# xyzy/jubatus

Hardware: AMD Instinct MI355X
Metric: train_samples_per_sec (higher is better)
Workload: dtype fp32

## Files before the change

jubatus_amd/csrc/hip/jb_device.hpp:

```cpp
#pragma once
#include <hip/hip_runtime.h>
#include <stdint.h>

namespace jb {

constexpr uint64_t kFnvOffset = 0xcbf29ce484222325ull;
constexpr uint64_t kFnvPrime = 0x100000001b3ull;

__device__ __forceinline__ uint64_t fnv_bytes(uint64_t h, const uint8_t* p, int n) {
  for (int i = 0; i < n; ++i) {
    h ^= (uint64_t)p[i];
    h *= kFnvPrime;
  }
  return h;
}

__device__ __forceinline__ uint64_t fnv_byte(uint64_t h, uint8_t b) {
  h ^= (uint64_t)b;
  return h * kFnvPrime;
}

__device__ __forceinline__ int64_t hash_to_index(uint64_t h, uint64_t H) {
  h ^= h >> 29;
  h *= 0xbf58476d1ce4e5b9ull;
  h ^= h >> 32;
  return (int64_t)__umul64hi(h, H);
}

struct Reader {
  const uint8_t* p;
  const uint8_t* end;
  bool ok;
  __device__ __forceinline__ bool need(int64_t n) {
    if (!ok || end - p < n) { ok = false; return false; }
    return true;
  }
  __device__ __forceinline__ uint32_t be16() { uint32_t v = ((uint32_t)p[0] << 8) | p[1]; p += 2; return v; }
  __device__ __forceinline__ uint32_t be32() {
    uint32_t v = ((uint32_t)p[0] << 24) | ((uint32_t)p[1] << 16) | ((uint32_t)p[2] << 8) | p[3];
    p += 4; return v;
  }
  __device__ __forceinline__ uint64_t be64() { uint64_t hi = be32(); uint64_t lo = be32(); return (hi << 32) | lo; }

  __device__ int64_t array_len() {
    if (!need(1)) return -1;
    uint8_t t = *p++;
    if ((t & 0xf0) == 0x90) return t & 0x0f;
    if (t == 0xdc) { if (!need(2)) return -1; return be16(); }
    if (t == 0xdd) { if (!need(4)) return -1; return be32(); }
    ok = false; return -1;
  }
  __device__ bool raw(const uint8_t** s, int* n) {
    if (!need(1)) return false;
    uint8_t t = *p++;
    int64_t len;
    if ((t & 0xe0) == 0xa0) len = t & 0x1f;
    else if (t == 0xd9 || t == 0xc4) { if (!need(1)) return false; len = *p++; }
    else if (t == 0xda || t == 0xc5) { if (!need(2)) return false; len = be16(); }
    else if (t == 0xdb || t == 0xc6) { if (!need(4)) return false; len = be32(); }
    else { ok = false; return false; }
    if (!need(len)) return false;
    *s = p; *n = (int)len; p += len;
    return true;
  }
  __device__ bool number(double* out) {
    if (!need(1)) return false;
    uint8_t t = *p++;
    if (t <= 0x7f) { *out = (double)t; return true; }
    if (t >= 0xe0) { *out = (double)(int8_t)t; return true; }
    switch (t) {
      case 0xcc: if (!need(1)) return false; *out = (double)(*p++); return true;
      case 0xcd: if (!need(2)) return false; *out = (double)be16(); return true;
      case 0xce: if (!need(4)) return false; *out = (double)be32(); return true;
      case 0xcf: if (!need(8)) return false; *out = (double)be64(); return true;
      case 0xd0: if (!need(1)) return false; *out = (double)(int8_t)(*p++); return true;
      case 0xd1: if (!need(2)) return false; *out = (double)(int16_t)be16(); return true;
      case 0xd2: if (!need(4)) return false; *out = (double)(int32_t)be32(); return true;
      case 0xd3: if (!need(8)) return false; *out = (double)(int64_t)be64(); return true;
      case 0xca: { if (!need(4)) return false; uint32_t u = be32(); *out = (double)__uint_as_float(u); return true; }
      case 0xcb: {
        if (!need(8)) return false;
        uint64_t u = be64();
        *out = __longlong_as_double((long long)u);
        return true;
      }
      default: ok = false; return false;
    }
  }
};

template <class T>
__device__ __forceinline__ void sys_store(T* p, T v) {
  __hip_atomic_store(p, v, __ATOMIC_RELAXED, __HIP_MEMORY_SCOPE_SYSTEM);
}
__device__ __forceinline__ void sys_stores_block_done() {
  asm volatile("s_waitcnt vmcnt(0)" ::: "memory");
  __syncthreads();
}

__device__ __forceinline__ float wave_sum(float v) {
#pragma unroll
  for (int off = 32; off > 0; off >>= 1) v += __shfl_xor(v, off, 64);
  return v;
}

enum : int {
  kDppXor1 = 0xB1,
  kDppXor2 = 0x4E,
  kDppRowRor8 = 0x128,
  kDppHalfMirror = 0x141,
  kDppMirror = 0x140,
};

template <int CTRL>
__device__ __forceinline__ float dpp_f(float v) {
  return __int_as_float(__builtin_amdgcn_update_dpp(0, __float_as_int(v), CTRL, 0xF, 0xF, false));
}
template <int CTRL>
__device__ __forceinline__ int dpp_i(int v) {
  return __builtin_amdgcn_update_dpp(0, v, CTRL, 0xF, 0xF, false);
}

__device__ __forceinline__ float partner16_f(float v, int lane) {
  auto r = __builtin_amdgcn_permlane16_swap(__float_as_uint(v), __float_as_uint(v), false, false);
  return __uint_as_float(((lane >> 4) & 1) ? r[0] : r[1]);
}
__device__ __forceinline__ int partner16_i(int v, int lane) {
  auto r = __builtin_amdgcn_permlane16_swap((unsigned)v, (unsigned)v, false, false);
  return (int)(((lane >> 4) & 1) ? r[0] : r[1]);
}
__device__ __forceinline__ float partner32_f(float v, int lane) {
  auto r = __builtin_amdgcn_permlane32_swap(__float_as_uint(v), __float_as_uint(v), false, false);
  return __uint_as_float(lane >= 32 ? r[0] : r[1]);
}
__device__ __forceinline__ int partner32_i(int v, int lane) {
  auto r = __builtin_amdgcn_permlane32_swap((unsigned)v, (unsigned)v, false, false);
  return (int)(lane >= 32 ? r[0] : r[1]);
}

__device__ __forceinline__ float row16_sum(float v) {
  v += dpp_f<kDppXor1>(v);
  v += dpp_f<kDppXor2>(v);
  v += dpp_f<kDppHalfMirror>(v);
  v += dpp_f<kDppMirror>(v);
  return v;
}

__device__ __forceinline__ float wave_sum_fast(float v, int lane) {
  v = row16_sum(v);
  v += partner16_f(v, lane);
  v += partner32_f(v, lane);
  return v;
}

}
```

jubatus_amd/csrc/hip/jb_linear.hpp:

```cpp
#pragma once
#include "jb_device.hpp"

namespace jb {

__device__ __forceinline__ float ld_agent(const float* p) {
  return __hip_atomic_load(p, __ATOMIC_RELAXED, __HIP_MEMORY_SCOPE_AGENT);
}

using bf16_t = uint16_t;

__device__ __forceinline__ uint32_t jb_mix32(uint32_t a, uint32_t b) {
  uint32_t h = a * 0x9E3779B1u ^ (b + 0x7F4A7C15u) * 0x85EBCA77u;
  h ^= h >> 15;
  h *= 0x2C1B3C6Du;
  h ^= h >> 12;
  h *= 0x297A2D39u;
  h ^= h >> 15;
  return h;
}

__device__ __forceinline__ float bf16_f(uint32_t b) { return __uint_as_float(b << 16); }

__device__ __forceinline__ uint32_t f_bf16_sr(float v, uint32_t r) {
  const uint32_t u = __float_as_uint(v);
  if ((u & 0x7f800000u) == 0x7f800000u) return (u >> 16) | ((u & 0xffffu) ? 0x40u : 0u);
  const uint32_t t = u + (r & 0xffffu);
  return t >> 16;
}

__device__ __forceinline__ float ldw(const float* p) { return ld_agent(p); }
__device__ __forceinline__ float ldw(const bf16_t* p) {
  const uint32_t* w = reinterpret_cast<const uint32_t*>((uintptr_t)p & ~(uintptr_t)3);
  const uint32_t v = __hip_atomic_load(w, __ATOMIC_RELAXED, __HIP_MEMORY_SCOPE_AGENT);
  return ((uintptr_t)p & 2) ? __uint_as_float(v & 0xffff0000u) : __uint_as_float(v << 16);
}
__device__ __forceinline__ void stw(float* p, float v, uint32_t) { *p = v; }
__device__ __forceinline__ void stw(bf16_t* p, float v, uint32_t r) { *p = (bf16_t)f_bf16_sr(v, r); }
__device__ __forceinline__ void addw(float* p, float d, uint32_t) { atomicAdd(p, d); }
__device__ __forceinline__ void addw(bf16_t* p, float d, uint32_t r) {
  uint32_t* w = reinterpret_cast<uint32_t*>((uintptr_t)p & ~(uintptr_t)3);
  const int sh = ((uintptr_t)p & 2) ? 16 : 0;
  uint32_t old = __hip_atomic_load(w, __ATOMIC_RELAXED, __HIP_MEMORY_SCOPE_AGENT);
  for (;;) {
    const float cur = bf16_f((old >> sh) & 0xffffu);
    const uint32_t nb = f_bf16_sr(cur + d, r);
    const uint32_t nw = (old & ~(0xffffu << sh)) | (nb << sh);
    if (nw == old) return;
    const uint32_t seen = atomicCAS(w, old, nw);
    if (seen == old) return;
    old = seen;
    r = jb_mix32(r, seen);
  }
}

enum Method : int { PERCEPTRON = 0, PA = 1, PA1 = 2, PA2 = 3, CW = 4, AROW = 5, NHERD = 6 };
enum UpdateMode : int { kExact = 0, kAtomic = 1, kHogwild = 2, kSerial = 3 };

__device__ __forceinline__ bool step_coeffs(int method, float margin, float var, float nrm,
                                            bool has_l, float C, float* tau, float* beta) {
  switch (method) {
    case PERCEPTRON:
      if (margin <= 0.f) { *tau = 1.f; *beta = 0.f; return true; }
      return false;
    case PA: case PA1: case PA2: {
      const float loss = 1.f - margin;
      if (!(loss > 0.f && nrm > 0.f)) return false;
      const float sq = (has_l ? 2.f : 1.f) * nrm;
      if (method == PA) *tau = loss / sq;
      else if (method == PA1) *tau = fminf(C, loss / sq);
      else *tau = loss / (sq + 0.5f / C);
      *beta = 0.f;
      return true;
    }
    case CW: {
      if (!(var > 0.f)) return false;
      const float phi = C;
      const float b = 1.f + 2.f * phi * margin;
      const float disc = b * b - 8.f * phi * (margin - phi * var);
      const float gamma = (-b + sqrtf(fmaxf(disc, 0.f))) / (4.f * phi * var);
      if (!(gamma > 0.f)) return false;
      *tau = gamma; *beta = 2.f * gamma * phi;
      return true;
    }
    case AROW:
      if (!(margin < 1.f)) return false;
      *beta = 1.f / (var + 1.f / C);
      *tau = (1.f - margin) * *beta;
      return true;
    case NHERD: {
      if (!(margin < 1.f)) return false;
      *tau = (1.f - margin) / (var + 1.f / C);
      const float cv = 1.f + C * var;
      *beta = (C * C * var + 2.f * C) / (cv * cv);
      return true;
    }
    default: return false;
  }
}

__device__ __forceinline__ float dprec(int method, float beta, float x, float s) {
  const float bx2 = beta * x * x;
  return method == CW ? bx2 : bx2 / (1.f - bx2 * s);
}

template <int LC>
struct Lanes {
  static constexpr int LW = LC >= 64 ? 64 : LC;
  static constexpr int G = 64 / LW;
  static constexpr int K = LC >= 64 ? LC / 64 : 1;
};

template <int LC, typename WT>
__device__ __forceinline__ void sample_scores(const int32_t* __restrict__ fidx,
                                              const float* __restrict__ fval, int64_t beg,
                                              int n, const WT* W, int lane, float (&acc)[Lanes<LC>::K]) {
  using L = Lanes<LC>;
  const int g = lane / L::LW;
  const int l0 = lane % L::LW;
#pragma unroll
  for (int k = 0; k < L::K; ++k) acc[k] = 0.f;
  for (int j = g; j < n; j += L::G) {
    const int32_t idx = fidx[beg + j];
    const float x = fval[beg + j];
    if (idx >= 0) {
      const WT* wr = W + (int64_t)idx * LC + l0;
#pragma unroll
      for (int k = 0; k < L::K; ++k) acc[k] += x * ldw(wr + 64 * k);
    }
  }
#pragma unroll
  for (int off = L::LW; off < 64; off <<= 1) {
#pragma unroll
    for (int k = 0; k < L::K; ++k) acc[k] += __shfl_xor(acc[k], off, 64);
  }
}

template <int LW>
__device__ __forceinline__ void argmax_wrong(float& best, int& bl) {
#pragma unroll
  for (int off = 1; off < LW; off <<= 1) {
    const float ob = __shfl_xor(best, off, 64);
    const int ol = __shfl_xor(bl, off, 64);
    if (ol >= 0 && (bl < 0 || ob > best || (ob == best && ol < bl))) { best = ob; bl = ol; }
  }
}

template <int LC, int MODE, typename WT>
__device__ __forceinline__ void apply_feature(WT* W, float* P, int32_t idx, float x, int y,
                                              int lstar, bool use_s, int method, float tau,
                                              float beta, float a, float b, float wy, float wl,
                                              uint32_t rnd) {
  const int64_t row = (int64_t)idx * LC;
  const float dwy = use_s ? tau * a * x : tau * x;
  const float dwl = use_s ? -tau * b * x : -tau * x;
  if (MODE == kAtomic) {
    addw(W + row + y, dwy, jb_mix32((uint32_t)(row + y), rnd));
    if (lstar >= 0) addw(W + row + lstar, dwl, jb_mix32((uint32_t)(row + lstar), rnd));
    if (use_s) {
      atomicAdd(P + row + y, dprec(method, beta, x, a));
      if (lstar >= 0) atomicAdd(P + row + lstar, dprec(method, beta, x, b));
    }
  } else {
    stw(W + row + y, wy + dwy, jb_mix32((uint32_t)(row + y), rnd));
    if (lstar >= 0) stw(W + row + lstar, wl + dwl, jb_mix32((uint32_t)(row + lstar), rnd));
    if (use_s) {
      P[row + y] = 1.f / a + dprec(method, beta, x, a);
      if (lstar >= 0) P[row + lstar] = 1.f / b + dprec(method, beta, x, b);
    }
  }
}

template <int LC, int MODE, typename WT>
__device__ __forceinline__ bool general_sample(const int32_t* __restrict__ fidx,
                                               const float* __restrict__ fval, int64_t beg, int n,
                                               int y, WT* W, float* P, const bool (&act)[Lanes<LC>::K],
                                               int lane, int method, float C,
                                               uint8_t* __restrict__ touched) {
  using L = Lanes<LC>;
  const int l0 = lane % L::LW;
  const bool use_s = method >= CW;
  float acc[L::K];
  sample_scores<LC>(fidx, fval, beg, n, W, lane, acc);
  float sy = 0.f, best = -INFINITY;
  int bl = -1;
#pragma unroll
  for (int k = 0; k < L::K; ++k) {
    const int l = l0 + 64 * k;
// ... 59 lines not shown
```

jubatus_amd/csrc/hip/linear.hip:

```cpp
#include "jb_linear.hpp"

namespace jb {

template <int LC, int MODE, typename WT>
__global__ __launch_bounds__(256) void linear_train_wide_kernel(
    const int64_t* __restrict__ row_ptr, const int32_t* __restrict__ fidx,
    const float* __restrict__ fval, const int32_t* __restrict__ labels,
    const int64_t* __restrict__ stream_ptr, int nstreams, WT* W, float* P,
    const int32_t* __restrict__ active, int method, float C,
    unsigned long long* __restrict__ stats, uint8_t* __restrict__ touched) {
  using L = Lanes<LC>;
  const int lane = threadIdx.x & 63;
  const int wid = (blockIdx.x * blockDim.x + threadIdx.x) >> 6;
  if (wid >= nstreams) return;
  bool act[L::K];
#pragma unroll
  for (int k = 0; k < L::K; ++k) act[k] = active[lane % L::LW + 64 * k] != 0;
  unsigned n_upd = 0, n_valid = 0;
  for (int64_t s = stream_ptr[wid]; s < stream_ptr[wid + 1]; ++s) {
    const int y = labels[s];
    if (y < 0 || y >= LC) continue;
    ++n_valid;
    const int64_t beg = row_ptr[s];
    if (general_sample<LC, MODE, WT>(fidx, fval, beg, (int)(row_ptr[s + 1] - beg), y, W, P, act, lane,
                                 method, C, touched))
      ++n_upd;
    if (MODE == kExact) asm volatile("s_waitcnt vmcnt(0)" ::: "memory");
  }
  if (stats != nullptr && lane == 0 && n_valid > 0) {
    atomicAdd(stats, (unsigned long long)n_upd);
    atomicAdd(stats + 1, (unsigned long long)n_valid);
  }
}

#ifndef JB_KREP
#define JB_KREP 8
#endif
constexpr int kRep = JB_KREP;

template <int LC>
struct Hot {
  static constexpr int E = 512;
  static constexpr int R = (E / LC) < 64 ? (E / LC) : 64;
  static constexpr int T = 128;
};

__device__ __forceinline__ int hot_find(const int32_t* hK, const int32_t* hS, int32_t idx) {
  if (idx < 0) return -1;
  uint32_t h = ((uint32_t)idx * 0x9E3779B1u) >> 25;
  for (int p = 0; p < 128; ++p) {
    const int32_t k = hK[h];
    if (k == idx) return hS[h];
    if (k < 0) return -1;
    h = (h + 1) & 127;
  }
  return -1;
}

template <int LC, int NW>
struct HotMerge {
  static constexpr int KQ = 2 * Hot<LC>::E / 64 / NW;
  float d[KQ];
  float own[KQ];
  float oth[KQ][kRep - 1];
  bool pending = false;

  template <int E>
  __device__ __forceinline__ void issue(const float* rep, int rr, bool use_s, int nent,
                                        float (*hA)[E], int wv, int lane) {
#pragma unroll
    for (int k = 0; k < KQ; ++k) {
      const int q = wv + NW * k;
      const int t = q & 1;
      const int e = (q >> 1) * 64 + lane;
      if (e < nent && (t == 0 || use_s)) {
        float* sh = const_cast<float*>(rep) + (int64_t)(rr * 2 + t) * E + e;
        d[k] = atomicExch(&hA[t][e], 0.f);
        own[k] = d[k] != 0.f ? atomicAdd(sh, d[k]) : ld_agent(sh);
#pragma unroll
        for (int j = 0; j < kRep - 1; ++j) {
          const int r = j < rr ? j : j + 1;
          oth[k][j] = ld_agent(rep + (int64_t)(r * 2 + t) * E + e);
        }
      }
    }
    pending = true;
  }

  template <int E>
  __device__ __forceinline__ void finish(bool use_s, int nent, float (*hV)[E], float (*hB)[E],
                                         float* hD, int wv, int lane) {
    if (!pending) return;
#pragma unroll
    for (int k = 0; k < KQ; ++k) {
      const int q = wv + NW * k;
      const int t = q & 1;
      const int e = (q >> 1) * 64 + lane;
      if (e < nent && (t == 0 || use_s)) {
        float S = own[k] + d[k];
#pragma unroll
        for (int j = 0; j < kRep - 1; ++j) S += oth[k][j];
        const float others = S - hB[t][e] - d[k];
        atomicAdd(&hV[t][e], others);
        if (t == 1) hD[e] = others;
        hB[t][e] = S;
      }
    }
    pending = false;
  }
};

template <int LC>
__global__ __launch_bounds__(256) void hot_fold_kernel(float* W, float* P, int use_s,
                                                       const int32_t* __restrict__ hot_rows,
                                                       const int32_t* __restrict__ hot_n,
                                                       float* __restrict__ rep,
                                                       uint8_t* __restrict__ touched) {
  constexpr int E = Hot<LC>::E;
  const int nh = min(*hot_n, Hot<LC>::R);
  const int i = blockIdx.x * blockDim.x + threadIdx.x;
  const int e = i % E;
  const int t = i / E;
  if (e >= nh * LC || t > 1 || (t == 1 && !use_s)) return;
  float s = 0.f;
#pragma unroll
  for (int r = 0; r < kRep; ++r) {
    float* p = rep + (int64_t)(r * 2 + t) * E + e;
    s += *p;
    *p = 0.f;
  }
  const int32_t row = hot_rows[e / LC];
  float* T = t == 0 ? W : P;
  if (s != 0.f) T[(int64_t)row * LC + (e % LC)] += s;
  if (touched != nullptr && t == 0 && e % LC == 0) touched[row] = 1;
}

template <int LC>
struct Pipe {
  static_assert(LC <= 64, "pipelined path covers label capacities up to 64");
  static constexpr int G = 64 / LC;
  static constexpr int F = LC <= 32 ? 32 : 16;
  static constexpr int U = F / G;
};

__device__ __forceinline__ int64_t readlane64(int64_t v, int i) {
  const int lo = __builtin_amdgcn_readlane((int)(uint32_t)(uint64_t)v, i);
  const int hi = __builtin_amdgcn_readlane((int)((uint64_t)v >> 32), i);
  return (int64_t)(((uint64_t)(uint32_t)hi << 32) | (uint32_t)lo);
}

__device__ __forceinline__ float readlane_f(float v, int i) {
  return __int_as_float(__builtin_amdgcn_readlane(__float_as_int(v), i));
}
// ... 288 lines not shown
      const float nrm = wave_sum_fast(x2s, lane);
      float tau = 0.f, beta = 0.f;
      upd = step_coeffs(method, margin, var, nrm, lstar >= 0, C, &tau, &beta);
      if (upd) ++n_upd;
      if (upd && mine) {
        dwy = use_s ? tau * a * x_s : tau * x_s;
        dwl = use_s ? -tau * b * x_s : -tau * x_s;
        if (use_s) {
          dpy = dprec(method, beta, x_s, a);
          dpl = lstar >= 0 ? dprec(method, beta, x_s, b) : 0.f;
        }
      }
      if (MODE == kAtomic && use_s && upd) {
        bool dup = false;
        for (int j = 0; j < n_s; ++j) {
          const int32_t ij = __builtin_amdgcn_readlane(idx_s, j);
          dup |= mine && j != lane && ij == idx_s;
        }
        tau_s = tau;
        ser = mine && !dup;
        if (ser && !(HOT && hs_s >= 0)) {
          const int64_t row = (int64_t)idx_s * LC;
          dwy = tau * x_s / atomicAdd(P + row + y_s, dpy);
          if (lstar >= 0) dwl = -tau * x_s / atomicAdd(P + row + lstar, dpl);
          p_done = true;
        }
      }
    }
    if (early) {
      gather_commit<LC>(sW[wv][c1], sP[wv][c1], use_s, n1, g, l0, vmask, gw, gp);
      if (upd) {
        float fwy = 0.f, fwl = 0.f, fpy = 0.f, fpl = 0.f;
        const bool kv = lane < n1 && idx1 >= 0 && hs1 < 0;
        for (int j = 0; j < n_s; ++j) {
          const int32_t ij = __builtin_amdgcn_readlane(idx_s, j);
          const bool hit = kv && ij == idx1;
          if (__builtin_amdgcn_ballot_w64(hit)) {
            const float ay = readlane_f(dwy, j);
            const float al = readlane_f(dwl, j);
            const float by = readlane_f(dpy, j);
            const float bq = readlane_f(dpl, j);
            if (hit) { fwy += ay; fwl += al; fpy += by; fpl += bq; }
          }
        }
        __builtin_amdgcn_wave_barrier();
        if (kv && (fwy != 0.f || fwl != 0.f || fpy != 0.f || fpl != 0.f)) {
          float* nw = sW[wv][c1] + lane * LC;
          float* np = sP[wv][c1] + lane * LC;
          nw[y_s] += fwy;
          if (lstar >= 0) nw[lstar] += fwl;
          if (use_s) {
            np[y_s] += fpy;
            if (lstar >= 0) np[lstar] += fpl;
          }
        }
      }
      __builtin_amdgcn_wave_barrier();
    }
    JB_CONSUME(idx2);
    JB_CONSUME(x2);
    const int hs2 = (HOT && nent > 0) ? hot_find(hK, hS, idx2) : -1;
    bool skip = false;
    if (MODE != kAtomic && upd) {
      float cy = 0.f, cl = 0.f, qy = 0.f, ql = 0.f;
      const bool plain = mine && hs_s < 0;
      for (int j = 0; j < n_s; ++j) {
        const int32_t ij = __builtin_amdgcn_readlane(idx_s, j);
        const bool same = plain && ij == idx_s && j != lane;
        if (__builtin_amdgcn_ballot_w64(same)) {
          const float ay = readlane_f(dwy, j);
          const float al = readlane_f(dwl, j);
          const float by = readlane_f(dpy, j);
          const float bq = readlane_f(dpl, j);
          if (same) {
            if (j < lane) skip = true;
            else { cy += ay; cl += al; qy += by; ql += bq; }
          }
        }
      }
      dwy += cy; dwl += cl; dpy += qy; dpl += ql;
    }
    if (upd && mine && !skip) {
      if (HOT && hs_s >= 0) {
        const int hb = hs_s * LC;
        if (use_s) {
          const float p0 = atomicAdd(&hV[1][hb + y_s], dpy);
          atomicAdd(&hA[1][hb + y_s], dpy);
          if (MODE == kAtomic && ser) dwy = tau_s * x_s / (p0 + hD[hb + y_s]);
          if (lstar >= 0) {
            const float q0 = atomicAdd(&hV[1][hb + lstar], dpl);
            atomicAdd(&hA[1][hb + lstar], dpl);
            if (MODE == kAtomic && ser) dwl = -tau_s * x_s / (q0 + hD[hb + lstar]);
          }
        }
        atomicAdd(&hV[0][hb + y_s], dwy);
        atomicAdd(&hA[0][hb + y_s], dwy);
        if (lstar >= 0) {
          atomicAdd(&hV[0][hb + lstar], dwl);
          atomicAdd(&hA[0][hb + lstar], dwl);
        }
      } else {
        const int64_t row = (int64_t)idx_s * LC;
        const uint32_t ry = jb_mix32((uint32_t)(row + y_s), (uint32_t)s);
        const uint32_t rl = jb_mix32((uint32_t)(row + lstar), (uint32_t)s);
        if (MODE == kAtomic) {
          addw(W + row + y_s, dwy, ry);
          if (lstar >= 0) addw(W + row + lstar, dwl, rl);
          if (use_s && !p_done) {
            atomicAdd(P + row + y_s, dpy);
            if (lstar >= 0) atomicAdd(P + row + lstar, dpl);
          }
        } else {
          stw(W + row + y_s, wy + dwy, ry);
          if (lstar >= 0) stw(W + row + lstar, wl + dwl, rl);
          if (use_s) {
            P[row + y_s] = py + dpy;
            if (lstar >= 0) P[row + lstar] = pl + dpl;
          }
        }
        if (touched != nullptr) touched[idx_s] = 1;
      }
    }
    if (MODE == kExact && (upd || general_s)) asm volatile("s_waitcnt vmcnt(0)" ::: "memory");
    if (pipe1 && !early) {
      if (MODE != kExact) asm volatile("s_waitcnt vmcnt(0)" ::: "memory");
      vmask = gather_issue<LC, WT>(W, P, use_s, sI[wv][c1], n1, g, l0, gw, gp);
      gather_commit<LC>(sW[wv][c1], sP[wv][c1], use_s, n1, g, l0, vmask, gw, gp);
    }
    put_features<LC>(sI[wv][c], sX[wv][c], idx2, hs2, x2, n2, lane);
    __builtin_amdgcn_wave_barrier();
    staged = pipe1;
    idx_s = idx1; x_s = x1; n_s = n1; y_s = y1; hs_s = hs1;
    idx1 = idx2; x1 = x2; n1 = n2; y1 = y2; hs1 = hs2;
  }
  if constexpr (HOT) mrg.template finish<HE>(use_s, nent, hV, hB, hD, wv, lane);
  }
  if (stats != nullptr && lane == 0 && n_valid > 0) {
    atomicAdd(stats, (unsigned long long)n_upd);
    atomicAdd(stats + 1, (unsigned long long)n_valid);
  }
  if (HOT) {
    __syncthreads();
    for (int e = threadIdx.x; e < nent; e += blockDim.x) {
      const float dw = hA[0][e];
      if (dw != 0.f) atomicAdd(hot_rep + (int64_t)(rr * 2) * HE + e, dw);
      if (use_s) {
        const float dp = hA[1][e];
        if (dp != 0.f) atomicAdd(hot_rep + (int64_t)(rr * 2 + 1) * HE + e, dp);
      }
    }
  }
}

template <int LC, typename WT>
__global__ __launch_bounds__(256) void linear_classify_kernel(
    const int64_t* __restrict__ row_ptr, const int32_t* __restrict__ fidx,
    const float* __restrict__ fval, int n_samples, const WT* W, float* __restrict__ out) {
  using L = Lanes<LC>;
  const int lane = threadIdx.x & 63;
  const int s = (blockIdx.x * blockDim.x + threadIdx.x) >> 6;
  if (s >= n_samples) return;
  const int64_t beg = row_ptr[s];
  const int n = (int)(row_ptr[s + 1] - beg);
  float acc[L::K];
  sample_scores<LC>(fidx, fval, beg, n, W, lane, acc);
  if (lane < L::LW) {
#pragma unroll
    for (int k = 0; k < L::K; ++k) out[(int64_t)s * LC + lane + 64 * k] = acc[k];
  }
}

__global__ void scale_kernel(float* __restrict__ p, int64_t n, float a) {
  const int64_t tid = (int64_t)blockIdx.x * blockDim.x + threadIdx.x;
  const int64_t stride = (int64_t)gridDim.x * blockDim.x * 4;
  const int64_t n4 = n & ~(int64_t)3;
  for (int64_t i = tid * 4; i < n4; i += stride) {
    float4 v = *reinterpret_cast<float4*>(p + i);
    v.x *= a; v.y *= a; v.z *= a; v.w *= a;
    *reinterpret_cast<float4*>(p + i) = v;
  }
  if (tid < n - n4) p[n4 + tid] *= a;
}

__global__ void mix_apply_kernel(float* __restrict__ w, const float* __restrict__ red,
                                 const float* __restrict__ loc, int64_t n, float inv_n) {
  const int64_t tid = (int64_t)blockIdx.x * blockDim.x + threadIdx.x;
  const int64_t stride = (int64_t)gridDim.x * blockDim.x;
  const int64_t n4 = n >> 2;
  float4* w4 = reinterpret_cast<float4*>(w);
  const float4* r4 = reinterpret_cast<const float4*>(red);
  const float4* l4 = reinterpret_cast<const float4*>(loc);
  for (int64_t i = tid; i < n4; i += stride) {
    float4 a = w4[i];
    const float4 r = r4[i], l = l4[i];
    a.x += r.x * inv_n - l.x; a.y += r.y * inv_n - l.y;
    a.z += r.z * inv_n - l.z; a.w += r.w * inv_n - l.w;
    w4[i] = a;
  }
  for (int64_t i = (n4 << 2) + tid; i < n; i += stride) w[i] += red[i] * inv_n - loc[i];
}

}

extern "C" int64_t jb_serial_scratch_bytes(int64_t n_max);
extern "C" int jb_serial_prepare(const int64_t* row_ptr, const int32_t* fidx, const float* fval,
                                 const int32_t* labels, const int64_t* stream_ptr, int nstreams,
                                 int64_t n_max, float* W, float* S, const int32_t* active, int LC,
                                 int method, float C, unsigned long long* stats, uint8_t* touched,
                                 void* scratch, int64_t scratch_bytes, int bail_after,
                                 hipStream_t stream);
extern "C" int jb_stepper_train(const int64_t* row_ptr, const int32_t* fidx, const float* fval,
                                const int32_t* labels, const int64_t* range, float* W, float* P,
                                const int32_t* active, int LC, int method, float C, unsigned long long* stats,
                                uint8_t* touched, int* err, hipStream_t stream);
extern "C" int jb_stepper_enabled();
constexpr int kSerialBail = 128;

namespace jb {

__global__ void stream_span_kernel(const int64_t* __restrict__ sp, int nstreams,
                                   int64_t* __restrict__ out) {
  if (threadIdx.x == 0) {
    out[0] = sp[0];
    out[1] = sp[nstreams];
  }
}

template <typename WT, int L, int M>
void launch_train(const int64_t* row_ptr, const int32_t* fidx, const float* fval,
                  const int32_t* labels, const int64_t* stream_ptr, int nstreams, WT* W, float* S,
                  const int32_t* active, int method, float C, bool hot, int hot_nw,
                  const int32_t* hot_rows, const int32_t* hot_n, float* hot_rep, int merge_every,
                  unsigned long long* stats, uint8_t* touched, hipStream_t stream) {
  const int threads = 256;
  const int blocks = (nstreams * 64 + threads - 1) / threads;
  const int hblocks = (nstreams + hot_nw - 1) / hot_nw;
#define JB_PIPE(H, NWV, B)                                                                      \
  hipLaunchKernelGGL((linear_train_pipe_kernel<L, M, H, NWV, WT>), dim3(B), dim3(64 * NWV), 0,  \
                     stream, row_ptr, fidx, fval, labels, stream_ptr, nstreams, W, S, active,   \
                     method, C, hot_rows, hot_n, hot_rep, merge_every, stats, touched);
  if constexpr (L <= 64) {
    if constexpr (M != kExact && sizeof(WT) == 4) {
      if (hot) {
        if constexpr (L <= 16) {
          if (hot_nw == 16) { JB_PIPE(true, 16, hblocks) return; }
        }
        if (hot_nw == 4) { JB_PIPE(true, 4, hblocks) }
        else { JB_PIPE(true, 8, hblocks) }
        return;
      }
    }
    JB_PIPE(false, 4, blocks)
  } else {
    hipLaunchKernelGGL((linear_train_wide_kernel<L, M, WT>), dim3(blocks), dim3(threads), 0, stream,
                       row_ptr, fidx, fval, labels, stream_ptr, nstreams, W, S, active, method, C,
                       stats, touched);
  }
#undef JB_PIPE
}

template <typename WT, int L>
void launch_train_mode(int mode, const int64_t* row_ptr, const int32_t* fidx, const float* fval,
                       const int32_t* labels, const int64_t* stream_ptr, int nstreams, WT* W,
                       float* S, const int32_t* active, int method, float C, bool hot, int hot_nw,
                       const int32_t* hot_rows, const int32_t* hot_n, float* hot_rep,
                       int merge_every, unsigned long long* stats, uint8_t* touched,
                       hipStream_t stream) {
#define JB_ARGS row_ptr, fidx, fval, labels, stream_ptr, nstreams, W, S, active, method, C, hot, \
                hot_nw, hot_rows, hot_n, hot_rep, merge_every, stats, touched, stream
  if (mode == kAtomic) launch_train<WT, L, kAtomic>(JB_ARGS);
  else if (mode == kHogwild) launch_train<WT, L, kHogwild>(JB_ARGS);
  else launch_train<WT, L, kExact>(JB_ARGS);
#undef JB_ARGS
}

}

template <typename WT>
static int linear_train_impl(const int64_t* row_ptr, const int32_t* fidx, const float* fval,
                             const int32_t* labels, const int64_t* stream_ptr, int nstreams,
                             WT* W, float* S, const int32_t* active, int LC, int method, float C,
                             int mode, const int32_t* hot_rows, const int32_t* hot_n,
                             float* hot_rep, int merge_every, int hot_waves,
                             unsigned long long* stats, uint8_t* touched, int64_t n_max,
                             void* scratch, int64_t scratch_bytes, hipStream_t stream) {
  if (nstreams <= 0) return 0;
  if (mode == jb::kSerial && nstreams == 1) mode = jb::kExact;
  if (mode == jb::kExact && nstreams > 1) mode = jb::kSerial;
  if (mode == jb::kSerial) {
    if constexpr (sizeof(WT) == 4) {
      const int rc = jb_serial_prepare(row_ptr, fidx, fval, labels, stream_ptr, nstreams, n_max,
                                       W, S, active, LC, method, C, stats, touched, scratch,
                                       scratch_bytes, kSerialBail, stream);
      if (rc != 0) return rc;
    } else {
      if (scratch == nullptr || scratch_bytes < 16) return -3;
      hipLaunchKernelGGL(jb::stream_span_kernel, dim3(1), dim3(64), 0, stream, stream_ptr,
                         nstreams, (int64_t*)scratch);
    }
    stream_ptr = (const int64_t*)scratch;
    nstreams = 1;
    mode = jb::kExact;
    hot_rows = nullptr;
  }
  if constexpr (sizeof(WT) == 4) {
    if (mode == jb::kExact && nstreams == 1 && LC <= 64 && jb_stepper_enabled())
      return jb_stepper_train(row_ptr, fidx, fval, labels, stream_ptr, W, S, active, LC, method, C,
                              stats, touched, nullptr, stream);
  }
  const bool hot = sizeof(WT) == 4 && hot_rows != nullptr && hot_n != nullptr &&
                   hot_rep != nullptr && mode != jb::kExact && LC <= 64;
  if (merge_every < 1) merge_every = 1;
  const int hot_nw = (hot_waves == 16 && LC <= 16) ? 16 : (hot_waves == 4 ? 4 : 8);
#define JB_TRAIN(L)                                                                             \
  jb::launch_train_mode<WT, L>(mode, row_ptr, fidx, fval, labels, stream_ptr, nstreams, W, S,   \
                               active, method, C, hot, hot_nw, hot_rows, hot_n, hot_rep,        \
                               merge_every, stats, touched, stream);
  JB_LC_DISPATCH(LC, JB_TRAIN)
#undef JB_TRAIN
  if constexpr (sizeof(WT) == 4) {
    if (hot) {
#define JB_FOLD(L)                                                                            \
  hipLaunchKernelGGL((jb::hot_fold_kernel<(L <= 64 ? L : 64)>), dim3(2 * jb::Hot<64>::E / 256), \
                     dim3(256), 0, stream, W, S, method >= jb::CW ? 1 : 0, hot_rows, hot_n,     \
                     hot_rep, touched);
      JB_LC_DISPATCH(LC, JB_FOLD)
#undef JB_FOLD
    }
  }
  return (int)hipGetLastError();
}

extern "C" int jb_linear_train(const int64_t* row_ptr, const int32_t* fidx, const float* fval,
                               const int32_t* labels, const int64_t* stream_ptr, int nstreams,
                               float* W, float* S, const int32_t* active, int LC, int method,
                               float C, int mode, const int32_t* hot_rows, const int32_t* hot_n,
                               float* hot_rep, int merge_every, int hot_waves,
                               unsigned long long* stats, uint8_t* touched, int64_t n_max,
                               void* scratch, int64_t scratch_bytes, hipStream_t stream) {
  return linear_train_impl<float>(row_ptr, fidx, fval, labels, stream_ptr, nstreams, W, S, active,
                                  LC, method, C, mode, hot_rows, hot_n, hot_rep, merge_every,
                                  hot_waves, stats, touched, n_max, scratch, scratch_bytes, stream);
}

extern "C" int jb_linear_train_bf16(const int64_t* row_ptr, const int32_t* fidx,
                                    const float* fval, const int32_t* labels,
                                    const int64_t* stream_ptr, int nstreams, jb::bf16_t* W,
                                    float* S, const int32_t* active, int LC, int method, float C,
                                    int mode, unsigned long long* stats, uint8_t* touched,
                                    void* scratch, int64_t scratch_bytes, hipStream_t stream) {
  return linear_train_impl<jb::bf16_t>(row_ptr, fidx, fval, labels, stream_ptr, nstreams, W, S,
                                       active, LC, method, C, mode, nullptr, nullptr, nullptr, 1,
                                       8, stats, touched, 0, scratch, scratch_bytes, stream);
}

extern "C" int64_t jb_hot_rep_bytes() { return (int64_t)jb::kRep * 2 * jb::Hot<8>::E * 4; }

template <typename WT>
static int linear_classify_impl(const int64_t* row_ptr, const int32_t* fidx, const float* fval,
                                int n_samples, const WT* W, int LC, float* out,
                                hipStream_t stream) {
  if (n_samples <= 0) return 0;
  const int threads = 256;
  const int blocks = (n_samples * 64 + threads - 1) / threads;
#define JB_CLS(L)                                                                           \
  hipLaunchKernelGGL((jb::linear_classify_kernel<L, WT>), dim3(blocks), dim3(threads), 0, \
                     stream, row_ptr, fidx, fval, n_samples, W, out);
  JB_LC_DISPATCH(LC, JB_CLS)
#undef JB_CLS
  return (int)hipGetLastError();
}

extern "C" int jb_linear_classify(const int64_t* row_ptr, const int32_t* fidx, const float* fval,
                                  int n_samples, const float* W, int LC, float* out,
                                  hipStream_t stream) {
  return linear_classify_impl<float>(row_ptr, fidx, fval, n_samples, W, LC, out, stream);
}

extern "C" int jb_linear_classify_bf16(const int64_t* row_ptr, const int32_t* fidx,
                                       const float* fval, int n_samples, const jb::bf16_t* W,
                                       int LC, float* out, hipStream_t stream) {
  return linear_classify_impl<jb::bf16_t>(row_ptr, fidx, fval, n_samples, W, LC, out, stream);
}

extern "C" int jb_scale(float* p, int64_t n, float a, hipStream_t stream) {
  if (n <= 0) return 0;
  const int threads = 256;
  int64_t blocks = (n / 4 + threads - 1) / threads;
  if (blocks > 4096) blocks = 4096;
  if (blocks < 1) blocks = 1;
  hipLaunchKernelGGL(jb::scale_kernel, dim3((unsigned)blocks), dim3(threads), 0, stream, p, n, a);
  return (int)hipGetLastError();
}

extern "C" int jb_mix_apply(float* w, const float* red, const float* loc, int64_t n, float inv_n,
                            hipStream_t stream) {
  if (n <= 0) return 0;
  if (((uintptr_t)w | (uintptr_t)red | (uintptr_t)loc) & 15) return -2;
  const int threads = 256;
  int64_t blocks = (n / 4 + threads - 1) / threads;
  if (blocks > 8192) blocks = 8192;
  if (blocks < 1) blocks = 1;
  hipLaunchKernelGGL(jb::mix_apply_kernel, dim3((unsigned)blocks), dim3(threads), 0, stream, w, red,
                     loc, n, inv_n);
  return (int)hipGetLastError();
}
```

Baseline: 269.5 million.

## Add software-pipelined block-per-stream training kernel for wide label capacities

Adds a new training kernel for label capacities above 64 that assigns one block per stream. Each thread owns one or more label columns, and weight rows for the next sample are gathered into registers while the current sample is scored and updated. Updates to rows shared between consecutive samples are forwarded through shared memory rather than re-read, and per-sample metadata is staged in windows. It becomes the default path, with the old wide kernel kept behind an environment variable; the cost is heavy register use from the F×K arrays and one block per stream, which may limit occupancy.

```diff
diff --git a/jubatus_amd/csrc/hip/jb_device.hpp b/jubatus_amd/csrc/hip/jb_device.hpp
--- a/jubatus_amd/csrc/hip/jb_device.hpp
+++ b/jubatus_amd/csrc/hip/jb_device.hpp
@@ -153,4 +153,14 @@
   return v;
 }
 
+__device__ __forceinline__ float wave_sum_xor(float v, int lane) {
+  v += partner32_f(v, lane);
+  v += partner16_f(v, lane);
+  v += dpp_f<kDppRowRor8>(v);
+  v += dpp_f<0x124>(v);
+  v += dpp_f<kDppXor2>(v);
+  v += dpp_f<kDppXor1>(v);
+  return v;
 }
+
+}
diff --git a/jubatus_amd/csrc/hip/jb_linear.hpp b/jubatus_amd/csrc/hip/jb_linear.hpp
--- a/jubatus_amd/csrc/hip/jb_linear.hpp
+++ b/jubatus_amd/csrc/hip/jb_linear.hpp
@@ -33,6 +33,14 @@
   const uint32_t* w = reinterpret_cast<const uint32_t*>((uintptr_t)p & ~(uintptr_t)3);
   const uint32_t v = __hip_atomic_load(w, __ATOMIC_RELAXED, __HIP_MEMORY_SCOPE_AGENT);
   return ((uintptr_t)p & 2) ? __uint_as_float(v & 0xffff0000u) : __uint_as_float(v << 16);
+}
+__device__ __forceinline__ float ldw_at(const float* W, int64_t base, int col) {
+  return ld_agent(W + base + col);
+}
+__device__ __forceinline__ float ldw_at(const bf16_t* W, int64_t base, int col) {
+  const uint32_t* w = reinterpret_cast<const uint32_t*>(W) + (base >> 1) + (col >> 1);
+  const uint32_t v = __hip_atomic_load(w, __ATOMIC_RELAXED, __HIP_MEMORY_SCOPE_AGENT);
+  return (col & 1) ? __uint_as_float(v & 0xffff0000u) : __uint_as_float(v << 16);
 }
 __device__ __forceinline__ void stw(float* p, float v, uint32_t) { *p = v; }
 __device__ __forceinline__ void stw(bf16_t* p, float v, uint32_t r) { *p = (bf16_t)f_bf16_sr(v, r); }
diff --git a/jubatus_amd/csrc/hip/linear.hip b/jubatus_amd/csrc/hip/linear.hip
--- a/jubatus_amd/csrc/hip/linear.hip
+++ b/jubatus_amd/csrc/hip/linear.hip
@@ -1,4 +1,7 @@
 #include "jb_linear.hpp"
+
+#include <cstdlib>
+#include <cstring>
 
 namespace jb {
 
@@ -593,6 +596,383 @@
   }
 }
 
+template <int LC>
+struct WidePipe {
+  static_assert(LC > 64, "label capacities up to 64 run linear_train_pipe_kernel");
+  static constexpr int T = LC <= 512 ? LC : 256;
+  static constexpr int K = LC / T;
+  static constexpr int NW = T / 64;
+  static constexpr int F = 16;
+  static constexpr int WIN = 64;
+};
+
+template <int LC, int MODE, typename WT>
+__global__ __launch_bounds__(WidePipe<LC>::T) void linear_train_wide_pipe_kernel(
+    const int64_t* __restrict__ row_ptr, const int32_t* __restrict__ fidx,
+    const float* __restrict__ fval, const int32_t* __restrict__ labels,
+    const int64_t* __restrict__ stream_ptr, int nstreams, WT* W, float* P,
+    const int32_t* __restrict__ active, int method, float C,
+    unsigned long long* __restrict__ stats, uint8_t* __restrict__ touched) {
+  using Q = WidePipe<LC>;
+  constexpr int T = Q::T, K = Q::K, NW = Q::NW, F = Q::F, WIN = Q::WIN;
+  static_assert(F == 16, "the match maps below split a wave into 4 x 16 lanes");
+  __shared__ int64_t dRP[WIN + 1];
+  __shared__ int32_t dLab[WIN];
+  __shared__ int32_t sI[2][F];
+  __shared__ float sX[2][F];
+  __shared__ int32_t sN[2];
+  __shared__ int32_t sY[2];
+  __shared__ int64_t sBeg[2];
+  __shared__ float sBest[NW];
+  __shared__ int32_t sBl[NW];
+  __shared__ float sSy;
+  __shared__ float sRow[4][F];
+  __shared__ float sInc[4][F];
+  __shared__ float sFwd[4][F];
+  __shared__ uint32_t sM[2];
+  __shared__ int32_t sUpd;
+  const int tid = threadIdx.x;
+  const int lane = tid & 63;
+  const int wv = tid >> 6;
+  const bool use_s = method >= CW;
+  if ((int)blockIdx.x >= nstreams) return;
+  const int64_t s_beg = stream_ptr[blockIdx.x];
+  const int64_t s_end = stream_ptr[blockIdx.x + 1];
+  if (s_beg >= s_end) return;
+  bool act[K];
+#pragma unroll
+  for (int k = 0; k < K; ++k) act[k] = active[tid + T * k] != 0;
+
+  int64_t wb = s_beg;
+  auto load_window = [&]() {
+    for (int i = tid; i <= WIN; i += T) {
+      dRP[i] = (wb + i <= s_end) ? row_ptr[wb + i] : 0;
+      if (i < WIN) dLab[i] = (wb + i < s_end) ? labels[wb + i] : -1;
+    }
+    __syncthreads();
+  };
+  auto fetch = [&](int64_t t, int& n, int& y, int64_t& beg, int32_t& idx, float& x) {
+    n = 0; y = -1; beg = 0; idx = -1; x = 0.f;
+    if (t < s_end) {
+      const int i = (int)(t - wb);
+      beg = dRP[i];
+      n = (int)(dRP[i + 1] - beg);
+      y = dLab[i];
+      if (lane < n && lane < F) {
+        idx = fidx[beg + lane];
+        x = fval[beg + lane];
+      }
+    }
+  };
+  auto put = [&](int slot, int n, int y, int64_t beg, int32_t idx, float x) {
+    const bool v = lane < F && lane < n && idx >= 0;
+    const uint32_t m = (uint32_t)__builtin_amdgcn_ballot_w64(v);
+    if (lane < F) {
+      sI[slot][lane] = v ? idx : -1;
+      sX[slot][lane] = v ? x : 0.f;
+    }
+    if (lane == 0) { sN[slot] = n; sY[slot] = y; sBeg[slot] = beg; sM[slot] = m; }
+  };
+  float cw[F][K], cp[F][K];
+  float gw[F][K], gp[F][K];
+  auto gather_rows = [&](const int32_t* si) {
+    int64_t rows[F];
+#pragma unroll
+    for (int j = 0; j < F; ++j) {
+      const int32_t idx = __builtin_amdgcn_readfirstlane(si[j]);
+      rows[j] = (int64_t)(idx >= 0 ? idx : 0) * LC;
+    }
+    if (use_s) {
+#pragma unroll
+      for (int j = 0; j < F; ++j) {
+#pragma unroll
+        for (int k = 0; k < K; ++k) {
+          gw[j][k] = ldw_at(W, rows[j], tid + T * k);
+          gp[j][k] = ld_agent(P + rows[j] + (tid + T * k));
+        }
+      }
+    } else {
+#pragma unroll
+      for (int j = 0; j < F; ++j) {
+#pragma unroll
+        for (int k = 0; k < K; ++k) {
+          gw[j][k] = ldw_at(W, rows[j], tid + T * k);
+          gp[j][k] = 1.f;
+        }
+      }
+    }
+  };
+  auto take_rows = [&](int slot) {
+    const uint32_t m = __builtin_amdgcn_readfirstlane(sM[slot]);
+#pragma unroll
+    for (int j = 0; j < F; ++j) {
+      const bool v = (m >> j) & 1u;
+#pragma unroll
+      for (int k = 0; k < K; ++k) {
+        cw[j][k] = v ? gw[j][k] : 0.f;
+        cp[j][k] = v ? gp[j][k] : 1.f;
+      }
+    }
+  };
+
+  load_window();
+  if (wv == 0) {
+    int n, y; int64_t beg; int32_t idx; float x;
+    fetch(s_beg, n, y, beg, idx, x);
+    put(0, n, y, beg, idx, x);
+    fetch(s_beg + 1, n, y, beg, idx, x);
+    put(1, n, y, beg, idx, x);
+  }
+  __syncthreads();
+  bool staged = sN[0] <= F;
+#pragma unroll
+  for (int j = 0; j < F; ++j) {
+#pragma unroll
+    for (int k = 0; k < K; ++k) { cw[j][k] = 0.f; cp[j][k] = 1.f; gw[j][k] = 0.f; gp[j][k] = 1.f; }
+  }
+  if (staged) {
+    gather_rows(sI[0]);
+    take_rows(0);
+  }
+  unsigned n_upd = 0, n_valid = 0;
+
+  for (int64_t s = s_beg; s < s_end; ++s) {
+    const int c = (int)((s - s_beg) & 1);
+    const int c1 = c ^ 1;
+    if (s + 3 - wb > WIN) {
+      wb = s;
+      load_window();
+    }
+    const int n_s = sN[c];
+    const int y_s = sY[c];
+    const int n1 = sN[c1];
+    const bool valid_s = y_s >= 0 && y_s < LC;
+    const bool general_s = valid_s && !staged;
+    const bool pipe1 = s + 1 < s_end && n1 <= F;
+    const bool early = pipe1 && !general_s;
+    int n2 = 0, y2 = -1;
+    int64_t beg2 = 0;
+    int32_t idx2 = -1;
+    float x2 = 0.f;
+    if (wv == 0) fetch(s + 2, n2, y2, beg2, idx2, x2);
+    if (early) gather_rows(sI[c1]);
+    bool upd = false;
+    int lstar = -1;
+    if (general_s) {
+      __syncthreads();
+      if (wv == 0) {
+        using L = Lanes<LC>;
+        bool actg[L::K];
+#pragma unroll
+        for (int k = 0; k < L::K; ++k) actg[k] = active[lane + 64 * k] != 0;
+        if (general_sample<LC, MODE, WT>(fidx, fval, sBeg[c], n_s, y_s, W, P, actg, lane, method, C,
+                                         touched))
+          ++n_upd;
+        ++n_valid;
+        asm volatile("s_waitcnt vmcnt(0)" ::: "memory");
+      }
+#pragma unroll
+      for (int j = 0; j < F; ++j) {
+#pragma unroll
+        for (int k = 0; k < K; ++k) { cw[j][k] = 0.f; cp[j][k] = 1.f; gw[j][k] = 0.f; gp[j][k] = 1.f; }
+      }
+    } else if (valid_s) {
+      float acc[K];
+#pragma unroll
+      for (int k = 0; k < K; ++k) acc[k] = 0.f;
+#pragma unroll
+      for (int j = 0; j < F; ++j) {
+        const float x = readlane_f(sX[c][j], 0);
+#pragma unroll
+        for (int k = 0; k < K; ++k) acc[k] += x * cw[j][k];
+      }
+      float best = -INFINITY;
+      int bl = -1;
+#pragma unroll
+      for (int k = 0; k < K; ++k) {
+        const int l = tid + T * k;
+        if (l == y_s) sSy = acc[k];
+        if (act[k] && l != y_s && acc[k] > best) { best = acc[k]; bl = l; }
+      }
+      group_argmax<64>(best, bl, lane);
+      if (lane == 0) { sBest[wv] = best; sBl[wv] = bl; }
+      __syncthreads();
+      best = sBest[0];
+      bl = sBl[0];
+#pragma unroll
+      for (int w = 1; w < NW; ++w) {
+        const float ob = sBest[w];
+        const int ol = sBl[w];
+        if (ol >= 0 && (bl < 0 || ob > best || (ob == best && ol < bl))) { best = ob; bl = ol; }
+      }
+      lstar = bl;
+      const float margin = sSy - (lstar >= 0 ? best : 0.f);
+#pragma unroll
+      for (int k = 0; k < K; ++k) {
+        const int l = tid + T * k;
+        if (l == y_s || l == lstar) {
+          const int t = l == y_s ? 0 : 1;
+#pragma unroll
+          for (int j = 0; j < F; ++j) {
+            sRow[t][j] = cw[j][k];
+            sRow[2 + t][j] = cp[j][k];
+          }
+        }
+      }
+      __syncthreads();
+      if (wv == 0) {
+        ++n_valid;
+        const int32_t idx_s = lane < F ? sI[c][lane] : -1;
+        const bool mine = idx_s >= 0;
+        const float x_s = mine ? sX[c][lane] : 0.f;
+        float wy = 0.f, wl = 0.f, py = 1.f, pl = 1.f, a = 1.f, b = 1.f, x2s = 0.f;
+        if (mine) {
+          x2s = x_s * x_s;
+          wy = sRow[0][lane];
+          wl = lstar >= 0 ? sRow[1][lane] : 0.f;
+          if (use_s) {
+            py = sRow[2][lane];
+            pl = lstar >= 0 ? sRow[3][lane] : 1.f;
+            a = 1.f / py;
+            b = lstar >= 0 ? 1.f / pl : 0.f;
+          }
+        }
+        const float var = use_s ? wave_sum_fast(x2s * (a + b), lane) : 0.f;
+        const float nrm = wave_sum_fast(x2s, lane);
+        float tau = 0.f, beta = 0.f;
+        upd = step_coeffs(method, margin, var, nrm, lstar >= 0, C, &tau, &beta);
+        float dwy = 0.f, dwl = 0.f, dpy = 0.f, dpl = 0.f;
+        if (upd) {
+          ++n_upd;
+          if (mine) {
+            dwy = use_s ? tau * a * x_s : tau * x_s;
+            dwl = lstar >= 0 ? (use_s ? -tau * b * x_s : -tau * x_s) : 0.f;
+            if (use_s) {
+              dpy = dprec(method, beta, x_s, a);
+              dpl = lstar >= 0 ? dprec(method, beta, x_s, b) : 0.f;
+            }
+          }
+          const int jk = lane & (F - 1);
+          const int jq = lane >> 4;
+          if (early) {
+            if (lane < F) {
+              sInc[0][lane] = dwy;
+              sInc[1][lane] = dwl;
+              sInc[2][lane] = dpy;
+              sInc[3][lane] = dpl;
+            }
+            __builtin_amdgcn_wave_barrier();
+            const int32_t idx1 = sI[c1][jk];
+            float fwy = 0.f, fwl = 0.f, fpy = 0.f, fpl = 0.f;
+#pragma unroll
+            for (int t = 0; t < F / 4; ++t) {
+              const int j = jq * (F / 4) + t;
+              const bool hit = idx1 >= 0 && sI[c][j] == idx1;
+              fwy += hit ? sInc[0][j] : 0.f;
+              fwl += hit ? sInc[1][j] : 0.f;
+              fpy += hit ? sInc[2][j] : 0.f;
+              fpl += hit ? sInc[3][j] : 0.f;
+            }
+            fwy += partner16_f(fwy, lane); fwy += partner32_f(fwy, lane);
+            fwl += partner16_f(fwl, lane); fwl += partner32_f(fwl, lane);
+            fpy += partner16_f(fpy, lane); fpy += partner32_f(fpy, lane);
+            fpl += partner16_f(fpl, lane); fpl += partner32_f(fpl, lane);
+            if (lane < F) {
+              sFwd[0][lane] = fwy;
+              sFwd[1][lane] = fwl;
+              sFwd[2][lane] = fpy;
+              sFwd[3][lane] = fpl;
+            }
+          }
+          bool skip = false;
+          bool rep_row = false;
+          if (MODE != kAtomic) {
+            const int32_t ia = sI[c][jk];
+#pragma unroll
+            for (int t = 0; t < F / 4; ++t) {
+              const int j = jq * (F / 4) + t;
+              rep_row |= ia >= 0 && j != jk && sI[c][j] == ia;
+            }
+          }
+          if (MODE != kAtomic && __builtin_amdgcn_ballot_w64(rep_row) != 0) {
+            float cy = 0.f, cl = 0.f, qy = 0.f, ql = 0.f;
+            for (int j = 0; j < n_s; ++j) {
+              const int32_t ij = __builtin_amdgcn_readlane(idx_s, j);
+              const bool same = mine && ij == idx_s && j != lane;
+              if (__builtin_amdgcn_ballot_w64(same)) {
+                const float ay = readlane_f(dwy, j);
+                const float al = readlane_f(dwl, j);
+                const float by = readlane_f(dpy, j);
+                const float bq = readlane_f(dpl, j);
+                if (same) {
+                  if (j < lane) skip = true;
+                  else { cy += ay; cl += al; qy += by; ql += bq; }
+                }
+              }
+            }
+            dwy += cy; dwl += cl; dpy += qy; dpl += ql;
+          }
+          if (mine && !skip) {
+            const int64_t row = (int64_t)idx_s * LC;
+            const uint32_t rnd = (uint32_t)sBeg[c];
+            const uint32_t ry = jb_mix32((uint32_t)(row + y_s), rnd);
+            const uint32_t rl = jb_mix32((uint32_t)(row + lstar), rnd);
+            if (MODE == kAtomic) {
+              addw(W + row + y_s, dwy, ry);
+              if (lstar >= 0) addw(W + row + lstar, dwl, rl);
+              if (use_s) {
+                atomicAdd(P + row + y_s, dpy);
+                if (lstar >= 0) atomicAdd(P + row + lstar, dpl);
+              }
+            } else {
+              stw(W + row + y_s, wy + dwy, ry);
+              if (lstar >= 0) stw(W + row + lstar, wl + dwl, rl);
+              if (use_s) {
+                P[row + y_s] = py + dpy;
+                if (lstar >= 0) P[row + lstar] = pl + dpl;
+              }
+            }
+            if (touched != nullptr) touched[idx_s] = 1;
+          }
+          if (MODE == kExact) asm volatile("s_waitcnt vmcnt(0)" ::: "memory");
+        }
+      }
+    } else {
+      __syncthreads();
+    }
+    if (wv == 0) {
+      if (lane == 0) sUpd = upd ? 1 : 0;
+      put(c, n2, y2, beg2, idx2, x2);
+    }
+    __syncthreads();
+    if (early) {
+      take_rows(c1);
+      if (sUpd != 0) {
+#pragma unroll
+        for (int k = 0; k < K; ++k) {
+          const int l = tid + T * k;
+          if (l == y_s || l == lstar) {
+            const int t = l == y_s ? 0 : 1;
+#pragma unroll
+            for (int j = 0; j < F; ++j) {
+              cw[j][k] += sFwd[t][j];
+              cp[j][k] += sFwd[2 + t][j];
+            }
+          }
+        }
+      }
+    } else if (pipe1) {
+      gather_rows(sI[c1]);
+      take_rows(c1);
+    }
+    staged = pipe1;
+  }
+  if (stats != nullptr && tid == 0 && n_valid > 0) {
+    atomicAdd(stats, (unsigned long long)n_upd);
+    atomicAdd(stats + 1, (unsigned long long)n_valid);
+  }
+}
+
 template <int LC, typename WT>
 __global__ __launch_bounds__(256) void linear_classify_kernel(
     const int64_t* __restrict__ row_ptr, const int32_t* __restrict__ fidx,
@@ -693,9 +1073,18 @@
     }
     JB_PIPE(false, 4, blocks)
   } else {
-    hipLaunchKernelGGL((linear_train_wide_kernel<L, M, WT>), dim3(blocks), dim3(threads), 0, stream,
-                       row_ptr, fidx, fval, labels, stream_ptr, nstreams, W, S, active, method, C,
-                       stats, touched);
+    static const bool direct = [] {
+      const char* e = getenv("JB_WIDE_LC");
+      return e != nullptr && strcmp(e, "direct") == 0;
+    }();
+    if (direct)
+      hipLaunchKernelGGL((linear_train_wide_kernel<L, M, WT>), dim3(blocks), dim3(threads), 0, stream,
+                         row_ptr, fidx, fval, labels, stream_ptr, nstreams, W, S, active, method, C,
+                         stats, touched);
+    else
+      hipLaunchKernelGGL((linear_train_wide_pipe_kernel<L, M, WT>), dim3(nstreams),
+                         dim3(WidePipe<L>::T), 0, stream, row_ptr, fidx, fval, labels, stream_ptr,
+                         nstreams, W, S, active, method, C, stats, touched);
   }
 #undef JB_PIPE
 }
```

After: 259.5 million. 0.963x the previous value.
